# shunkenney/DPE-MVS

Hardware: AMD Instinct MI355X
Metric: depth-map Mpixels/sec (9-view 1600x1200 PatchMatch) at 1/2/4/8 GPUs; L1 vs ref (higher is better)
Workload: dtype f32; 1 GPU; DTU-like 1600x1200, 9 src views, full-res REFINE_ITER pass + geometric consistency (BASELINE configs[2]); width=1600, height=1200, num_images=10, parallelism=reference-image sharding x1

## Files before the change

### dpe-mvs_amd/csrc/dpe_mvs.hip

```cpp
#include <hip/hip_runtime.h>
#include <rocprofiler-sdk-roctx/roctx.h>
#include <algorithm>
#include <cmath>
#include <cstdio>
#include <cstring>
#include <string>
#include <atomic>
#include <map>
#include <memory>
#include <mutex>
#include <utility>
#include <vector>

#include "pass_kernels.h"
#include "pass_refine.h"
#include "pass_fusion.h"
#include "pass_sweep.h"
#include "pass_edges.h"
#include "pass_viz.h"
#include "tap_launch.h"
#include "dpe_context.h"

using namespace dpe;

static const int kDefaultXcdRows = 1;
static constexpr int kWeakLanes = 16;

namespace {
// ... 168 lines not shown
    pc.vc[v].b[2] = (float)(sK8 * trel[2]);
  }
  pc.kinv0 = (float)(1.0 / rK0);
  pc.kinv4 = (float)(1.0 / rK4);
  pc.kc2 = (float)(rK2 / rK0);
  pc.kc5 = (float)(rK5 / rK4);
  const float angle = 45.0f / pc.P.rotate_time;
  pc.gn_cos = (float)cos((double)angle * M_PI / 180.f);
  pc.gn_sin = (float)sin((double)angle * M_PI / 180.f);
  pc.gn_thr = (float)cos((double)(angle / 2.0f) * M_PI / 180.0f);
  const double sr = tan((double)(angle / 2.0f) * M_PI / 180.0f) * 20;
  const int sri = (sr != sr) ? 0 : (int)sr;
  pc.gn_shift = sri < 1 ? 1 : sri;
  pc.half_rows = std::min(pc.H, 2 * 16 * (((pc.H / 2) + 15) / 16));
  pc.weak_nn = pc.P.weak_radius >= 0 && pc.P.weak_increment > 0 ? (2 * pc.P.weak_radius) / pc.P.weak_increment + 1 : 0;
}

#if DPE_POOL_STATS
extern "C" void dpe_dbg_pool_stats_main(unsigned long long out[24], int reset) {
  (void)hipMemcpyFromSymbol(out, HIP_SYMBOL(dpe::g_pool), sizeof(dpe::g_pool));
  if (reset) { unsigned long long z[24] = {}; (void)hipMemcpyToSymbol(HIP_SYMBOL(dpe::g_pool), z, sizeof(z)); }
}
#endif
#if DPE_LINE_STATS
extern "C" void dpe_dbg_line_stats_main(unsigned long long out[16], int reset) {
  (void)hipMemcpyFromSymbol(out, HIP_SYMBOL(dpe::g_lstat), sizeof(dpe::g_lstat));
  if (reset) { unsigned long long z[16] = {}; (void)hipMemcpyToSymbol(HIP_SYMBOL(dpe::g_lstat), z, sizeof(z)); }
}
#endif
#if DPE_GN_TIMES
// ... 1220 lines not shown
```

### dpe-mvs_amd/csrc/pass_common.h

```cpp
#pragma once
#include "device_math.h"
#include "bres_walk.h"
#include "../../include/dpe_mvs.h"

namespace dpe {

struct ViewConst { float M[9]; float b[3]; };

struct PassConst {
  int W, H, N, LW, LH;
  int half_rows;
  uint32_t seed32, salt;
  float kinv0, kinv4, kc2, kc5;
  float gn_cos, gn_sin, gn_thr;
  int gn_shift;
  uint32_t gn_shift_m;
  int weak_nn;
  DpePatchMatchParams P;
  DpeCamera cams[DPE_MAX_IMAGES];
  ViewConst vc[DPE_MAX_IMAGES];
};

struct DevBufs {
  const float4* imgq[DPE_MAX_IMAGES];
  const uint8_t* img8; uint32_t img8_view;
  const uint8_t* img16; uint32_t img16_view;
  const uint8_t* imgp; uint32_t imgp_view;
  const float* depth[DPE_MAX_IMAGES];
  const float* ref;
  float4* planes; float4* planes_snap; float4* fit_plane;
  const float4* planes0;
  float* costs; float* costs_snap; float* complex_;
  uint32_t* sel; uint32_t* sel_snap;
  uint8_t* weak; uint8_t* weak_rel; uint8_t* vw;
  short2* nb; short2* nearest; short2* edge_neigh; short2* lab_bound;
  int* radius;
  const uint8_t* edge; const uint8_t* edge_low; const int* label;
  unsigned long long* cnt;
  unsigned long long* phase;
  int xcd_rows;
};

#ifndef DPE_DIAG
#define DPE_DIAG 0
#endif
#ifndef DPE_UNCLAMPED
#define DPE_UNCLAMPED 1
#endif
#define DPE_POOL_STATS (((DPE_DIAG) >> 4) & 1)
#define DPE_PHASE_PROF ((DPE_DIAG) & 1)
#define DPE_LINE_STATS (((DPE_DIAG) >> 1) & 1)
#define DPE_WEAK_STATS (((DPE_DIAG) >> 2) & 1)
#define DPE_GN_TIMES (((DPE_DIAG) >> 3) & 1)
#define DPE_FAKE_GATHER (((DPE_DIAG) >> 5) & 1)
#define DPE_GN_ONCE (((DPE_DIAG) >> 6) & 1)
#if DPE_PHASE_PROF
#define PHASE_BEGIN() uint64_t ph_t_ = __builtin_readcyclecounter(), ph_acc_[16] = {}
#define PHASE(k)                                                                    \
  do {                                                                              \
    const uint64_t n_ = __builtin_readcyclecounter();                               \
    ph_acc_[k] += n_ - ph_t_;                                                       \
    ph_t_ = n_;                                                                     \
// ... 150 lines not shown
    q1 = 2.0f * u32_to_uniform(rng_word(rs, w)) - 1.0f;
    q2 = 2.0f * u32_to_uniform(rng_word(rs, w + 1)) - 1.0f;
    s = q1 * q1 + q2 * q2;
    w += 2;
  }
  const float sq = __builtin_sqrtf(1.0f - s);
  d.n[0] = 2.0f * q1 * sq; d.n[1] = 2.0f * q2 * sq; d.n[2] = 1.0f - 2.0f * s;
  d.u_pert = u32_to_uniform(rng_word(rs, w));
  d.w_angles = w + 1;
  return d;
}
DEV void refine_angle(const Rng& rs, uint32_t w_angles, int k, float pert, float* s, float* c) {
  const float a = (u32_to_uniform(rng_word(rs, w_angles + (uint32_t)k)) - 0.5f) * pert;
  d_sincosf(a, s, c);
}
DEV float4 random_normal_from(const DpeCamera& c, int px, int py, const float* n0, float depth) {
  float4 n = make_float4(n0[0], n0[1], n0[2], 0.0f);
  const float4 vd = view_direction(c, px, py, depth);
  if (n.x * vd.x + n.y * vd.y + n.z * vd.z > 0.0f) { n.x = -n.x; n.y = -n.y; n.z = -n.z; }
  normalize3(n);
  return n;
}
DEV float4 perturbed_normal_from(const DpeCamera& c, int px, int py, const float4& normal, const float* sc) {
  const float4 vd = view_direction(c, px, py, 1.0f);
  const float s1 = sc[0], c1 = sc[1], s2 = sc[2], c2 = sc[3], s3 = sc[4], c3 = sc[5];
  const float R0 = c2 * c3, R1 = c3 * s1 * s2 - c1 * s3, R2 = s1 * s3 + c1 * c3 * s2;
  const float R3 = c2 * s3, R4 = c1 * c3 + s1 * s2 * s3, R5 = c1 * s2 * s3 - c3 * s1;
  const float R6 = -s2, R7 = c2 * s1, R8 = c1 * c2;
  float4 np = make_float4(R0 * normal.x + R1 * normal.y + R2 * normal.z,
                          R3 * normal.x + R4 * normal.y + R5 * normal.z,
                          R6 * normal.x + R7 * normal.y + R8 * normal.z, normal.w);
  if (np.x * vd.x + np.y * vd.y + np.z * vd.z >= 0.0f) np = normal;
  normalize3(np);
  return np;
}

struct Homog { float h[9]; };
DEV Homog make_homography(const PassConst& pc, int v, const float4& pl) {
  const float iw = 1.0f / pl.w;
  const float qx = pl.x * iw, qy = pl.y * iw, qz = pl.z * iw;
  const float g0 = qx * pc.kinv0;
  const float g1 = qy * pc.kinv4;
  const float g2 = __builtin_fmaf(-qx, pc.kc2, __builtin_fmaf(-qy, pc.kc5, qz));
  const ViewConst& vc = pc.vc[v];
  Homog H;
  H.h[0] = __builtin_fmaf(-vc.b[0], g0, vc.M[0]);
  H.h[1] = __builtin_fmaf(-vc.b[0], g1, vc.M[1]);
  H.h[2] = __builtin_fmaf(-vc.b[0], g2, vc.M[2]);
  H.h[3] = __builtin_fmaf(-vc.b[1], g0, vc.M[3]);
// ... 245 lines not shown

template <int U8> DEV float sample_src(const DevBufs& B, int v, int W, int H, float Qx, float Qy, float iz) {
  if constexpr (U8 != TEX_F32) return sample_quad8<U8>(tex_base<U8>(B) + (size_t)v * tex_view<U8>(B), W, H, Qx, Qy, iz);
  else return sample_quad(B.imgq[v], W, H, Qx, Qy, iz);
}

DEV float depth_texel(const float* d, int W, int H, float x, float y) {
  return ref_texel(d, W, H, f2i(x), f2i(y));
}

DEV float bilateral_weight(int i, int j, float pix, float cpix, float ss, float sc) {
  const float xd = (float)i, yd = (float)j;
  const float sd = __builtin_sqrtf(xd * xd + yd * yd);
  const float cd = __builtin_fabsf(pix - cpix);
  return d_expf(-sd / (2.0f * ss * ss) - cd / (2.0f * sc * sc));
}

DEV void ncc_pre(float s_ref, float s_rr, float s_w, float& inv, float& mref, float& var_ref) {
  inv = 1.0f / s_w;
  mref = s_ref * inv;
  const float mrr = s_rr * inv;
  var_ref = mrr - mref * mref;
}
DEV float ncc_finalize_pre(float inv, float mref, float var_ref, float s_src, float s_ss, float s_rs) {
  s_src *= inv; s_ss *= inv; s_rs *= inv;
  const float var_src = s_ss - s_src * s_src;
  if (var_ref < 1e-5f || var_src < 1e-5f) return 2.0f;
  const float cov = s_rs - mref * s_src;
  const float vrs = __builtin_sqrtf(var_ref * var_src);
  return __builtin_fmaxf(0.0f, __builtin_fminf(2.0f, 1.0f - cov / vrs));
// ... 76 lines not shown
DEV float ncc_old_generic(const PassConst& pc, const DevBufs& B, int px, int py, int v, const float4& pl) {
  const Homog H = make_homography(pc, v, pl);
  count_work(B, 1, 0);
  if (center_outside(pc, v, H, px, py)) return 2.0f;
  const float rc = ref_texel(B.ref, pc.W, pc.H, px, py);
  return patch_ncc_generic<U8>(pc, B, v, H, px, py, rc, pc.P.strong_radius, pc.P.strong_increment);
}

struct Patch36 {
  float w[36], wr[36];
  float s_ref, s_rr, s_w;
  int px, py;
};
DEV void make_patch36(Patch36& P, const PassConst& pc, const DevBufs& B, int px, int py) {
  const int W = pc.W, Hh = pc.H;
  const float ss = pc.P.sigma_spatial, sc = pc.P.sigma_color;
  const float rc = ref_texel(B.ref, W, Hh, px, py);
  P.px = px; P.py = py;
  float s_ref = 0, s_rr = 0, s_w = 0;
#pragma unroll
  for (int a = 0; a < 6; ++a) {
    const int i = -5 + 2 * a;
    float r_ref = 0, r_rr = 0, r_w = 0;
#pragma unroll
    for (int b = 0; b < 6; ++b) {
      const int j = -5 + 2 * b;
      const float rp = ref_texel(B.ref, W, Hh, px + i, py + j);
      const float w = bilateral_weight(i, j, rp, rc, ss, sc);
      const float wr = w * rp;
      r_ref = r_ref + wr;
      r_rr = __builtin_fmaf(wr, rp, r_rr);
      r_w = r_w + w;
      P.w[a * 6 + b] = w;
      P.wr[a * 6 + b] = wr;
    }
    s_ref += r_ref; s_rr += r_rr; s_w += r_w;
  }
  P.s_ref = s_ref; P.s_rr = s_rr; P.s_w = s_w;
}
template <int U8>
DEV void patch36_taps(const Patch36& P, const PassConst& pc, const DevBufs& B, int v, const Homog& H0, float* acc) {
  const int W = pc.W, Hh = pc.H;
  const Homog H = scale_cols(H0);
// ... 159 lines not shown
```

### dpe-mvs_amd/csrc/pass_refine.h

```cpp
#pragma once
#include "pass_common.h"

namespace dpe {

DEV void wave_sync() {
  __builtin_amdgcn_fence(__ATOMIC_RELEASE, "wavefront");
  __builtin_amdgcn_wave_barrier();
  __builtin_amdgcn_fence(__ATOMIC_ACQUIRE, "wavefront");
}

template <int S>
DEV void patch_lds_build(float* pw, const PassConst& pc, const DevBufs& B, int px, int py, int t) {
  constexpr int R = (36 + S - 1) / S;
  const float rc = ref_texel(B.ref, pc.W, pc.H, px, py);
  float rp[R];
#pragma unroll
  for (int r = 0; r < R; ++r) {
    const int k = t + r * S < 36 ? t + r * S : 35;
    rp[r] = ref_texel(B.ref, pc.W, pc.H, px - 5 + 2 * (k / 6), py - 5 + 2 * (k % 6));
  }
#pragma unroll
  for (int r = 0; r < R; ++r) {
    const int k = t + r * S;
    if (k >= 36) break;
    const int i = -5 + 2 * (k / 6), j = -5 + 2 * (k % 6);
    const float w = bilateral_weight(i, j, rp[r], rc, pc.P.sigma_spatial, pc.P.sigma_color);
    pw[2 * k] = w;
    pw[2 * k + 1] = w * rp[r];
    pw[72 + k] = rp[r];
  }
}
DEV void patch_lds_pre(const float* pw, float& p_inv, float& p_mref, float& p_var) {
  float a_ref = 0, a_rr = 0, a_w = 0;
#pragma unroll
  for (int a = 0; a < 6; ++a) {
    float r_ref = 0, r_rr = 0, r_w = 0;
#pragma unroll
    for (int b = 0; b < 6; ++b) {
      const float w = pw[2 * (a * 6 + b)], wr = pw[2 * (a * 6 + b) + 1], rp = pw[72 + a * 6 + b];
      r_ref = r_ref + wr;
      r_rr = __builtin_fmaf(wr, rp, r_rr);
// ... 150 lines not shown
template <int U8>
DEV float ncc_old_any(bool fast, const float* pw, float s_ref, float s_rr, float s_w, int px, int py,
                      const PassConst& pc, const DevBufs& B, int v, const float4& pl) {
  if (fast) return ncc_old_lds<U8>(pw, s_ref, s_rr, s_w, px, py, pc, B, v, pl);
  return ncc_old_generic<U8>(pc, B, px, py, v, pl);
}

DEV void baseline_and_weights(const PassConst& pc, uint32_t sel, const uint8_t* vw, float& base_line, float& weight_normal,
                              int& valid) {
  const DpeCamera& c0 = pc.cams[0];
  base_line = 0.0f; weight_normal = 0.0f; valid = 0;
  for (int si = 1; si < pc.N; ++si) {
    const int vi = si - 1;
    if (isSet(sel, vi)) {
      weight_normal += vw[vi];
      const DpeCamera& cs = pc.cams[si];
      const float d0 = c0.c[0] - cs.c[0], d1 = c0.c[1] - cs.c[1], d2 = c0.c[2] - cs.c[2];
      const float tv = d0 * d0 + d1 * d1 + d2 * d2;
      base_line += __builtin_sqrtf(tv);
      valid++;
    }
  }
}

DEV uint8_t d2w_class(const PassConst& pc, const float* pcs, uint64_t is_peak) {
  const int radius = 30;
  const int peak_count = __popcll(is_peak);
  int min_peak = 0;
  float min_cost = 2.0f;
  for (uint64_t m = is_peak; m; m &= m - 1) {
    const int i = __builtin_ctzll(m);
    if (pcs[i] < min_cost) { min_peak = i; min_cost = pcs[i]; }
  }
  uint8_t cls;
// ... 22 lines not shown
DEV long border_pixel(long i, int W, int H) {
  constexpr int m = kD2WMargin;
  if (W <= 2 * m || H <= 2 * m) return i;
  const long top = (long)m * W;
  if (i < top) return i;
  if (i < 2 * top) return (long)(H - m) * W + (i - top);
  const long r = i - 2 * top;
  const int row = m + (int)(r / (2 * m)), c = (int)(r % (2 * m));
  return (long)row * W + (c < m ? c : W - 2 * m + c);
}
template <int U8, bool LR = false>
__global__ void __launch_bounds__(64 * kBwD2W, kTapWaves) k_depth_to_weak(const PassConst* __restrict__ pcp, DevBufs B) {
  __shared__ float s_patch[kBwD2W][108];
  __shared__ float s_pc[kBwD2W][64];
  __shared__ float s_lr[kBwD2W][11];
  const PassConst& pc = *pcp;
  const int wave = threadIdx.x >> 6, lane = threadIdx.x & 63;
  const int W = pc.W, H = pc.H;
  const long pix = (long)xcd_remap(blockIdx.x, gridDim.x, B.xcd_rows * 16 * ((pc.W + kBwD2W - 1) / kBwD2W)) * kBwD2W + wave;
  if (pix >= (long)W * H) return;
  const int x = (int)(pix % W), y = (int)(pix / W);
  const int center = (int)pix;
  const int min_margin = kD2WMargin;
  if (x < min_margin || y < min_margin || x >= W - min_margin || y >= H - min_margin) {
    if (lane == 0) B.weak[center] = DPE_UNKNOWN;
    return;
  }
  const DpeCamera& c0 = pc.cams[0];
  const float4 op = transform_normal_ref(c0, B.planes[center]);
  const float od = op.w;
  if (od == 0) { if (lane == 0) B.weak[center] = DPE_UNKNOWN; return; }
  PHASE_BEGIN();
  const uint32_t sel = B.sel[center];
  const uint8_t* vw = B.vw + (size_t)DPE_MAX_IMAGES * center;
  float base_line, weight_normal; int valid;
  baseline_and_weights(pc, sel, vw, base_line, weight_normal, valid);
  if (valid == 0) { if (lane == 0) B.weak[center] = DPE_UNKNOWN; return; }
// ... 29 lines not shown
          if constexpr (LR) lr += (c * vw[vi]);
          if (pc.P.geom_consistency) {
            const float g = pc.P.geom_factor * geom_cost_at(pc, B, x, y, si, fw);
            tcst += g;
            if constexpr (LR) lr += (g * vw[vi]);
          }
          PHASE(2);
          p_cost += (tcst * vw[vi]);
        }
      }
      p_cost /= weight_normal;
      val = lane == kNow ? p_cost : MINo(2.0f, p_cost);
      lr /= weight_normal;
    }
    s_pc[wave][lane] = val;
    if (LR && lane >= radius - 5 && lane <= radius + 5) s_lr[wave][lane - (radius - 5)] = lr;
  }
  wave_sync();
  PHASE(3);
  const float* pcs = s_pc[wave];
  const bool pk = lane >= 2 && lane < 59 && pcs[lane - 1] > pcs[lane] && pcs[lane + 1] > pcs[lane];
  const uint64_t is_peak = __ballot(pk);
  PHASE(4);
  PHASE_END(3);
  if (lane != 0) return;
  B.weak[center] = d2w_class(pc, pcs, is_peak);
  if (!lr_pix) return;
  float min_cost = 2.0f, best_depth = od;
  for (int pd = -5; pd <= 5; ++pd) {
    const float p_depth = c0.K[0] * base_line / (disp + (float)pd);
    if (p_depth < pc.P.depth_min || p_depth > pc.P.depth_max) continue;
    const float tcv = s_lr[wave][pd + 5];
    if (tcv < min_cost) { min_cost = tcv; best_depth = p_depth; }
  }
  if ((double)(pcs[kNow] - min_cost) > 0.1) B.planes[center].w = best_depth;
}

constexpr int kLrPix = 4;
template <int U8>
__global__ void __launch_bounds__(64 * kBwLR, kTapWaves) k_local_refine_jobs(const PassConst* __restrict__ pcp, DevBufs B,
                                                                                     int border) {
  constexpr int BW = kBwLR;
  __shared__ float s_patch[BW][kLrPix][108];
  __shared__ float s_sum[BW][kLrPix][3];
  __shared__ float4 s_hyp[BW][kLrPix][12];
// ... 180 lines not shown
```

### dpe-mvs_amd/csrc/pass_sweep.h

```cpp
#pragma once
#include "pass_common.h"
#include "pass_refine.h"
#include "lds_layout.h"

namespace dpe {

template <int MODE> constexpr int list_count() { return MODE == 0 ? 4 : 1; }
template <int MODE> DEV int list_rows(const PassConst& pc) { return MODE == 1 ? pc.H : pc.half_rows; }
template <int MODE> DEV int list_key(const PassConst& pc, const DevBufs& B, int x, int y) {
  if constexpr (MODE == 2) return (((x + y) & 1) == 0 && B.weak_rel[y * pc.W + x] == 0) ? 0 : -1;
  const bool wk = B.weak[y * pc.W + x] == DPE_WEAK;
  if constexpr (MODE == 1) return wk ? 0 : -1;
  else return (((x + y) & 1) << 1) | (wk ? 1 : 0);
}
template <int MODE>
__global__ void k_list_count(const PassConst* __restrict__ pcp, DevBufs B, int* __restrict__ row_counts) {
  constexpr int NL = list_count<MODE>();
  const PassConst& pc = *pcp;
  const int wave = threadIdx.x >> 6, lane = threadIdx.x & 63;
  const int y = blockIdx.x * 4 + wave, rows = list_rows<MODE>(pc);
  if (y >= rows) return;
  int cnt[NL];
  for (int j = 0; j < NL; ++j) cnt[j] = 0;
  for (int x0 = 0; x0 < pc.W; x0 += 64) {
// ... 288 lines not shown
      }
      return cmp;
    }
    default: {
      if (!(x < W - 1)) return -1;
      const int right_near = center + 1; costMin = costs[right_near]; cmp = right_near;
      for (int i = 0; i < 3; ++i) {
        if (x < W - 2 - i && y > i) { const int pt = right_near + (1 + i) - (1 + i) * W; if (costs[pt] < costMin) { costMin = costs[pt]; cmp = pt; } }
        if (x < W - 2 - i && y < H - 1 - i) { const int pt = right_near + (1 + i) + (1 + i) * W; if (costs[pt] < costMin) { costMin = costs[pt]; cmp = pt; } }
      }
      return cmp;
    }
  }
}

constexpr int kTailJobs = 16;
template <int P, int C> using StrongCarveT = lds::StrongCarve<P, C, kTailJobs>;
__host__ __device__ inline int strong_lds_per_wave(int P, int C, int nv) {
  return P == 4 && C == 16 ? StrongCarveT<4, 16>::total(nv) : StrongCarveT<8, 8>::total(nv);
}

template <int P>
DEV bool job_decode(const int* cnt, int j, int& p, int& r) {
  r = j;
#pragma unroll
  for (int q = 0; q < P; ++q) {
    if (r < cnt[q]) { p = q; return true; }
    r -= cnt[q];
  }
  return false;
}

constexpr int kBwStrong = 2;
template <int U8, bool EDGE>
__global__ void __launch_bounds__(64 * kBwStrong, kTapWaves) k_strong_coop(const PassConst* __restrict__ pcp, DevBufs B, int iter,
                                                     const int* __restrict__ list, const int* __restrict__ nlist_p) {
  extern __shared__ float4 lds4[];
  float* lds = (float*)lds4;
  const int nlist = *nlist_p;
  constexpr int C = EDGE ? 16 : 8;
  constexpr int P = 64 / C;
  const PassConst& pc = *pcp;
  const int wave = threadIdx.x >> 6, lane = threadIdx.x & 63;
  const int ps = lane / C, c = lane % C;
  const int W = pc.W, nv = pc.N - 1;
  const DpeCamera& c0 = pc.cams[0];
  const int wbase = (xcd_remap(blockIdx.x, gridDim.x, B.xcd_rows * 16) * kBwStrong + wave) * P;
  if (wbase >= nlist) return;
  const int gi = wbase + ps;
  const bool active = gi < nlist;
  const int center = active ? list[gi] : 0;
  const int x = center % W, y = center / W;
  using SC = StrongCarveT<P, C>;
  float* wl = lds + (size_t)wave * SC::total(nv);
  float4* hyp_all = (float4*)(wl + SC::hyp());
  float* pw_all = wl + SC::patch();
// ... 70 lines not shown
      while (m) {
        const int t = __builtin_ctz(m);
        if (same(cpl[t], me)) { a = t; break; }
        m &= m - 1;
      }
      al[r] = a;
    }
  }
  wave_sync();
  if (active) {
    alias[c] = al[0];
    if (c == 0) alias[C] = al[1];
  }
  wave_sync();
  PHASE(1);
  if (c == 0) {
    int n = 0;
    if (active) {
      for (int k = 0; k <= C; ++k) if (alias[k] == k) slots[n++] = k;
      if (fast) patch_lds_pre(pw, sums_all[ps * 4 + 0], sums_all[ps * 4 + 1], sums_all[ps * 4 + 2]);
    }
    misc[SC::MI_JOBS] = n;
  }
  wave_sync();
  PHASE(2);
  {
    int cnt[P], S = 0;
#pragma unroll
    for (int q = 0; q < P; ++q) { cnt[q] = ib_all[q * ibs + SC::IB_MISC + 1]; S += cnt[q]; }
    int q, r;
    const int total = S * nv, tail = total & 63;
    const bool split = fast && tail > 0 && tail <= kTailJobs;
    POOL_STAT(0, total);
    const int jend = split ? total - tail : total;
    for (int j = lane; j < jend; j += 64) {
      job_decode<P>(cnt, j % S, q, r);
      const int* iq = ib_all + q * ibs;
      const int slot = iq[SC::ib_slots(nv) + r], v = j / S + 1;
      const int cq = list[wbase + q];
      const int qx = cq % W, qy = cq / W;
      const float4 pl = cpl_all[q * (C + 1) + slot];
      const float* sm = sums_all + q * 4;
      cost_all[(q * (C + 1) + slot) * nv + v - 1] =
          ncc_old_any<U8>(fast, pw_all + q * 108, sm[0], sm[1], sm[2], qx, qy, pc, B, v, pl);
    }
    if (split) {
      float* tb = wl + SC::tail(nv);
      const int rpp = 64 / tail >= 6 ? 1 : 2, npc = 6 / rpp;
      if (lane < tail * npc) {
        const int j = jend + lane / npc, a0 = (lane % npc) * rpp;
        job_decode<P>(cnt, j % S, q, r);
        const int slot = ib_all[q * ibs + SC::ib_slots(nv) + r], v = j / S + 1;
        const int cq = list[wbase + q];
        const int qx = cq % W, qy = cq / W;
        const Homog H = make_homography(pc, v, cpl_all[q * (C + 1) + slot]);
        if (!center_outside(pc, v, H, qx, qy)) {
          const bool fr = rcp_range_ok(H, (float)(qx - 5), (float)(qx + 5), (float)(qy - 5), (float)(qy + 5));
          for (int a = a0; a < a0 + rpp; ++a) {
            float* r3 = tb + ((lane / npc) * 6 + a) * 3;
            if (fr) lds_row<U8, true>(pw_all + q * 108, qx, qy, pc, B, v, H, a, r3);
            else lds_row<U8, false>(pw_all + q * 108, qx, qy, pc, B, v, H, a, r3);
          }
        }
      }
      wave_sync();
      if (lane < tail) {
        const int j = jend + lane;
        job_decode<P>(cnt, j % S, q, r);
        const int slot = ib_all[q * ibs + SC::ib_slots(nv) + r], v = j / S + 1;
        const int cq = list[wbase + q];
        const Homog H = make_homography(pc, v, cpl_all[q * (C + 1) + slot]);
        float cst = 2.0f;
        if (center_outside(pc, v, H, cq % W, cq / W)) {
          count_work(B, 1, 0);
        } else {
          count_work(B, 1, 36);
          float s_src = 0, s_ss = 0, s_rs = 0;
          for (int a = 0; a < 6; ++a) {
            const float* r3 = tb + (lane * 6 + a) * 3;
            s_src += r3[0]; s_ss += r3[1]; s_rs += r3[2];
          }
          const float* sm = sums_all + q * 4;
          cst = ncc_finalize_pre(sm[0], sm[1], sm[2], s_src, s_ss, s_rs);
        }
        cost_all[(q * (C + 1) + slot) * nv + v - 1] = cst;
      }
    }
  }
  wave_sync();
  PHASE(3);
  if (active) {
    for (int sl = c; sl <= C; sl += C) {
      const int a = alias[sl];
      if (a >= 0 && a != sl)
        for (int v = 0; v < nv; ++v) cost[sl * nv + v] = cost[a * nv + v];
    }
  }
  wave_sync();
  PHASE(4);
  if (active && c < 8) {
    if constexpr (EDGE) {
      const int d = c;
// ... 36 lines not shown
    }
    for (int v = c; v < nv; v += C) {
      float prior = 0.0f;
#pragma unroll
      for (int i = 0; i < 4; ++i) if (nfl[i]) prior += isSet(nsv[i], v) == 1 ? 0.9f : 0.1f;
      sp[v] = view_prob_raw(cst, v, cost_threshold) * prior;
    }
  }
  wave_sync();
  PHASE(6);
  Rng rs;
  rng_init(rs, (uint32_t)center, pc.seed32, STREAM_ITER_BASE + 4 * iter + 0, pc.salt);
  view_sample_coop(sp, (int*)ref, nv, c, C, active, rs, vwl, B.vw + (size_t)center * DPE_MAX_IMAGES);
  PHASE(12);
  uint32_t tsv = 0; float wnorm = 0.0f;
  if (c == 0) {
    int ns = 0;
    if (active) {
      rng_seek(rs, 15);
      for (int i = 0; i < nv; ++i) if (vwl[i] > 0) { setBit(tsv, i); wnorm += vwl[i]; sel_list[ns++] = i; }
      sums_all[ps * 4 + 3] = wnorm;
    }
    misc[SC::MI_NSEL] = ns;
  }
  wave_sync();
  PHASE(7);
  const int nsel = active ? misc[SC::MI_NSEL] : 0;
  if (active && c < 8) {
    float wn = 0.0f;
    for (int i = 0; i < nv; ++i) wn += vwl[i];
    float f = 0.0f;
    for (int j = 0; j < nv; ++j) { const int w = vwl[j]; if (w > 0) f += w * cst(c, j); }
    fc[c] = f / wn;
  }
  wave_sync();
  PHASE(8);
  float cost_now = 0.0f, cost_written = 0.0f, depth_now = 0.0f;
  float4 pnow = make_float4(0, 0, 0, 0);
// ... 11 lines not shown
    cost_now /= wnorm;
    cost_written = cost_now;
    B.costs[center] = cost_now;
    depth_now = depth_from_plane(c0, curp, x, y);
    pnow = curp;
    const int f = fin[mi];
    if (f >= 0) {
      const float4 cand = planes_s[posl[f]];
      const float db = depth_from_plane(c0, cand, x, y);
      if (db >= pc.P.depth_min && db <= pc.P.depth_max && fc[mi] < cost_now) {
        depth_now = db; pnow = cand; cost_now = fc[mi]; B.sel[center] = tsv;
      }
    }
  }
  wave_sync();
  if (active && c == 0) {
    const float dmin = pc.P.depth_min, dmax = pc.P.depth_max;
    const float depth_rand = rnd[0] * (dmax - dmin) + dmin;
    const float4 prand = random_normal_from(c0, x, y, rnd + 1, depth_now);
    const float dminp = (1 - 0.02f) * depth_now, dmaxp = (1 + 0.02f) * depth_now;
    const float depth_perturbed = rnd[4] * (dmaxp - dminp) + dminp;
    const float4 ppert = perturbed_normal_from(c0, x, y, pnow, rnd + 5);
    float4 h0 = pnow, h1 = prand, h2 = prand, h3 = ppert, h4 = pnow;
    h0.w = dist2origin(c0, x, y, depth_rand, h0);
    h1.w = dist2origin(c0, x, y, depth_now, h1);
    h2.w = dist2origin(c0, x, y, depth_rand, h2);
    h3.w = dist2origin(c0, x, y, depth_now, h3);
    h4.w = dist2origin(c0, x, y, depth_perturbed, h4);
    hyp[0] = h0; hyp[1] = h1; hyp[2] = h2; hyp[3] = h3; hyp[4] = h4;
  }
  wave_sync();
  PHASE(9);
  {
    int cnt[P];
#pragma unroll
    for (int q = 0; q < P; ++q) cnt[q] = 5 * ib_all[q * ibs + SC::IB_MISC];
    POOL_STAT(1, [&] { int t = 0; for (int q = 0; q < P; ++q) t += cnt[q]; return t; }());
    int q, r;
    for (int j = lane; job_decode<P>(cnt, j, q, r); j += 64) {
      const int* iq = ib_all + q * ibs;
      const int h = r % 5, k = r / 5;
      const int cq = list[wbase + q];
      const float* sm = sums_all + q * 4;
      ref_all[(q * 5 + h) * nv + k] = ncc_old_any<U8>(fast, pw_all + q * 108, sm[0], sm[1], sm[2], cq % W, cq / W, pc,
                                                      B, iq[SC::IB_SEL + k] + 1, hyp_all[q * 5 + h]);
    }
  }
  wave_sync();
  PHASE(10);
  if (active && c < 5) {
    const int h = c;
    float tc = 0.0f;
    for (int k = 0; k < nsel; ++k) tc += vwl[sel_list[k]] * ref[h * nv + k];
    tc /= sums_all[ps * 4 + 3];
    fc[h] = tc;
    misc[SC::MI_DEPTH + h] = __float_as_int(depth_from_plane(c0, hyp[h], x, y));
  }
  wave_sync();
  PHASE(13);
  if (active && c == 0) {
    const float dmin = pc.P.depth_min, dmax = pc.P.depth_max;
// ... 645 lines not shown
```

### dpe-mvs_amd/csrc/tap_f32.hip

```cpp
#define DPE_TAP_TU 1
#include "tap_launch.h"
#include "pass_refine.h"
#include "pass_sweep.h"

namespace dpe {

void launch_strong_f32(bool edge, unsigned grid, size_t lds, hipStream_t s, const PassConst* dpc, const DevBufs& B,
                       int it, const int* list, const int* count) {
  constexpr int T = 64 * kBwStrong;
  if (lds > 65536) {
    static bool once = false;
    if (!once) {
      once = true;
      (void)hipFuncSetAttribute((const void*)k_strong_coop<TEX_F32, true>, hipFuncAttributeMaxDynamicSharedMemorySize, 160 * 1024);
      (void)hipFuncSetAttribute((const void*)k_strong_coop<TEX_F32, false>, hipFuncAttributeMaxDynamicSharedMemorySize, 160 * 1024);
    }
  }
  if (edge) k_strong_coop<TEX_F32, true><<<grid, T, lds, s>>>(dpc, B, it, list, count);
  else k_strong_coop<TEX_F32, false><<<grid, T, lds, s>>>(dpc, B, it, list, count);
}

void launch_depth_to_weak_f32(unsigned grid, hipStream_t s, const PassConst* dpc, const DevBufs& B) {
  k_depth_to_weak<TEX_F32, true><<<grid, 64 * kBwD2W, 0, s>>>(dpc, B);
}
// ... 6 lines not shown
      once = true;
      (void)hipFuncSetAttribute((const void*)k_local_refine_jobs<TEX_F32>, hipFuncAttributeMaxDynamicSharedMemorySize, 160 * 1024);
    }
  }
  k_local_refine_jobs<TEX_F32><<<grid, 64 * kBwLR, lds, s>>>(dpc, B, border);
}

}

#if DPE_POOL_STATS
extern "C" void dpe_dbg_pool_stats_f32(unsigned long long out[24], int reset) {
  (void)hipMemcpyFromSymbol(out, HIP_SYMBOL(dpe::g_pool), sizeof(dpe::g_pool));
  if (reset) { unsigned long long z[24] = {}; (void)hipMemcpyToSymbol(HIP_SYMBOL(dpe::g_pool), z, sizeof(z)); }
}
#endif
#if DPE_LINE_STATS
extern "C" void dpe_dbg_line_stats_f32(unsigned long long out[16], int reset) {
  (void)hipMemcpyFromSymbol(out, HIP_SYMBOL(dpe::g_lstat), sizeof(dpe::g_lstat));
  if (reset) { unsigned long long z[16] = {}; (void)hipMemcpyToSymbol(HIP_SYMBOL(dpe::g_lstat), z, sizeof(z)); }
}
#endif
```

### dpe-mvs_amd/csrc/tap_launch.hip

```cpp
#define DPE_TAP_TU 1
#include "tap_launch.h"
#include "pass_refine.h"
#include "pass_sweep.h"

namespace dpe {

void launch_strong(bool edge, int cls, unsigned grid, size_t lds, hipStream_t s, const PassConst* dpc,
                   const DevBufs& B, int it, const int* list, const int* count) {
  constexpr int T = 64 * kBwStrong;
  if (lds > 65536) {
    static bool once = false;
    if (!once) {
      once = true;
      (void)hipFuncSetAttribute((const void*)k_strong_coop<kTexStrong, true>, hipFuncAttributeMaxDynamicSharedMemorySize, 160 * 1024);
      (void)hipFuncSetAttribute((const void*)k_strong_coop<kTexStrong, false>, hipFuncAttributeMaxDynamicSharedMemorySize, 160 * 1024);
    }
  }
  if (cls == IMG_F32) { launch_strong_f32(edge, grid, lds, s, dpc, B, it, list, count); return; }
  if (edge) k_strong_coop<kTexStrong, true><<<grid, T, lds, s>>>(dpc, B, it, list, count);
  else k_strong_coop<kTexStrong, false><<<grid, T, lds, s>>>(dpc, B, it, list, count);
}

void launch_depth_to_weak(int cls, long L, hipStream_t s, const PassConst* dpc, const DevBufs& B) {
  const unsigned g = (unsigned)((L + kBwD2W - 1) / kBwD2W);
// ... 14 lines not shown
      (void)hipFuncSetAttribute((const void*)k_local_refine_jobs<kTexLR>, hipFuncAttributeMaxDynamicSharedMemorySize, 160 * 1024);
    }
  }
  if (cls == IMG_F32) { launch_local_refine_f32(g, lds, border, s, dpc, B); return; }
  k_local_refine_jobs<kTexLR><<<g, 64 * kBwLR, lds, s>>>(dpc, B, border);
}

}

#if DPE_POOL_STATS
extern "C" void dpe_dbg_pool_stats_tap(unsigned long long out[24], int reset) {
  (void)hipMemcpyFromSymbol(out, HIP_SYMBOL(dpe::g_pool), sizeof(dpe::g_pool));
  if (reset) { unsigned long long z[24] = {}; (void)hipMemcpyToSymbol(HIP_SYMBOL(dpe::g_pool), z, sizeof(z)); }
}
#endif
#if DPE_LINE_STATS
extern "C" void dpe_dbg_line_stats_tap(unsigned long long out[16], int reset) {
  (void)hipMemcpyFromSymbol(out, HIP_SYMBOL(dpe::g_lstat), sizeof(dpe::g_lstat));
  if (reset) { unsigned long long z[16] = {}; (void)hipMemcpyToSymbol(HIP_SYMBOL(dpe::g_lstat), z, sizeof(z)); }
}
#endif
```

Before: 30.68 Mpix/s.

## Precompute spatial weights and baselines, spread per-pixel serial work across lanes, widen tail split

Several independent changes. The host now precomputes the bilateral spatial term table and the per-view baseline lengths into PassConst, so the exp and sqrt inputs are no longer recomputed per tap or per pixel. Depth-to-weak caches candidate depths in LDS instead of recomputing a division. The strong cooperative kernel spreads work that lane 0 of each group did serially (slot compaction, selected-view list, building 5 hypotheses) across the group's lanes using ballot and popcount. The tail-job split is generalised into a helper that handles up to 32 leftover jobs and is also applied to the hypothesis-cost pool. These add shuffles and extra LDS use and more code paths, with A/B macros left in to disable each piece.

```diff
diff --git a/dpe-mvs_amd/csrc/dpe_mvs.hip b/dpe-mvs_amd/csrc/dpe_mvs.hip
--- a/dpe-mvs_amd/csrc/dpe_mvs.hip
+++ b/dpe-mvs_amd/csrc/dpe_mvs.hip
@@ -12,6 +12,7 @@
 #include <utility>
 #include <vector>
 
+#include "pass_tables.h"
 #include "pass_kernels.h"
 #include "pass_refine.h"
 #include "pass_fusion.h"
@@ -210,6 +211,8 @@
   pc.gn_shift = sri < 1 ? 1 : sri;
   pc.half_rows = std::min(pc.H, 2 * 16 * (((pc.H / 2) + 15) / 16));
   pc.weak_nn = pc.P.weak_radius >= 0 && pc.P.weak_increment > 0 ? (2 * pc.P.weak_radius) / pc.P.weak_increment + 1 : 0;
+  for (int v = 1; v < pc.N; ++v) pc.base_len[v] = baseline_length(rc.c, pc.cams[v].c);
+  build_spat36(pc.P.sigma_spatial, pc.spat36);
 }
 
 #if DPE_POOL_STATS
diff --git a/dpe-mvs_amd/csrc/pass_common.h b/dpe-mvs_amd/csrc/pass_common.h
--- a/dpe-mvs_amd/csrc/pass_common.h
+++ b/dpe-mvs_amd/csrc/pass_common.h
@@ -16,6 +16,8 @@
   int gn_shift;
   uint32_t gn_shift_m;
   int weak_nn;
+  float base_len[DPE_MAX_IMAGES];
+  float spat36[36];
   DpePatchMatchParams P;
   DpeCamera cams[DPE_MAX_IMAGES];
   ViewConst vc[DPE_MAX_IMAGES];
@@ -46,6 +48,9 @@
 #endif
 #ifndef DPE_UNCLAMPED
 #define DPE_UNCLAMPED 1
+#endif
+#ifndef DPE_AB_OFF
+#define DPE_AB_OFF 0
 #endif
 #define DPE_POOL_STATS (((DPE_DIAG) >> 4) & 1)
 #define DPE_PHASE_PROF ((DPE_DIAG) & 1)
@@ -226,15 +231,16 @@
   const float a = (u32_to_uniform(rng_word(rs, w_angles + (uint32_t)k)) - 0.5f) * pert;
   d_sincosf(a, s, c);
 }
-DEV float4 random_normal_from(const DpeCamera& c, int px, int py, const float* n0, float depth) {
+DEV float4 random_normal_vd(const float4& vd, const float* n0) {
   float4 n = make_float4(n0[0], n0[1], n0[2], 0.0f);
-  const float4 vd = view_direction(c, px, py, depth);
   if (n.x * vd.x + n.y * vd.y + n.z * vd.z > 0.0f) { n.x = -n.x; n.y = -n.y; n.z = -n.z; }
   normalize3(n);
   return n;
 }
-DEV float4 perturbed_normal_from(const DpeCamera& c, int px, int py, const float4& normal, const float* sc) {
-  const float4 vd = view_direction(c, px, py, 1.0f);
+DEV float4 random_normal_from(const DpeCamera& c, int px, int py, const float* n0, float depth) {
+  return random_normal_vd(view_direction(c, px, py, depth), n0);
+}
+DEV float4 perturbed_normal_vd(const float4& vd, const float4& normal, const float* sc) {
   const float s1 = sc[0], c1 = sc[1], s2 = sc[2], c2 = sc[3], s3 = sc[4], c3 = sc[5];
   const float R0 = c2 * c3, R1 = c3 * s1 * s2 - c1 * s3, R2 = s1 * s3 + c1 * c3 * s2;
   const float R3 = c2 * s3, R4 = c1 * c3 + s1 * s2 * s3, R5 = c1 * s2 * s3 - c3 * s1;
@@ -245,6 +251,9 @@
   if (np.x * vd.x + np.y * vd.y + np.z * vd.z >= 0.0f) np = normal;
   normalize3(np);
   return np;
+}
+DEV float4 perturbed_normal_from(const DpeCamera& c, int px, int py, const float4& normal, const float* sc) {
+  return perturbed_normal_vd(view_direction(c, px, py, 1.0f), normal, sc);
 }
 
 struct Homog { float h[9]; };
@@ -520,6 +529,14 @@
   const float sd = __builtin_sqrtf(xd * xd + yd * yd);
   const float cd = __builtin_fabsf(pix - cpix);
   return d_expf(-sd / (2.0f * ss * ss) - cd / (2.0f * sc * sc));
+}
+
+DEV float bilateral_weight36(const PassConst& pc, int k, float pix, float cpix) {
+  const float sc = pc.P.sigma_color;
+  if constexpr ((DPE_AB_OFF) & 2)
+    return bilateral_weight(-5 + 2 * (k / 6), -5 + 2 * (k % 6), pix, cpix, pc.P.sigma_spatial, sc);
+  const float cd = __builtin_fabsf(pix - cpix);
+  return d_expf(pc.spat36[k] - cd / (2.0f * sc * sc));
 }
 
 DEV void ncc_pre(float s_ref, float s_rr, float s_w, float& inv, float& mref, float& var_ref) {
@@ -626,7 +643,6 @@
 };
 DEV void make_patch36(Patch36& P, const PassConst& pc, const DevBufs& B, int px, int py) {
   const int W = pc.W, Hh = pc.H;
-  const float ss = pc.P.sigma_spatial, sc = pc.P.sigma_color;
   const float rc = ref_texel(B.ref, W, Hh, px, py);
   P.px = px; P.py = py;
   float s_ref = 0, s_rr = 0, s_w = 0;
@@ -638,7 +654,7 @@
     for (int b = 0; b < 6; ++b) {
       const int j = -5 + 2 * b;
       const float rp = ref_texel(B.ref, W, Hh, px + i, py + j);
-      const float w = bilateral_weight(i, j, rp, rc, ss, sc);
+      const float w = bilateral_weight36(pc, a * 6 + b, rp, rc);
       const float wr = w * rp;
       r_ref = r_ref + wr;
       r_rr = __builtin_fmaf(wr, rp, r_rr);
diff --git a/dpe-mvs_amd/csrc/pass_refine.h b/dpe-mvs_amd/csrc/pass_refine.h
--- a/dpe-mvs_amd/csrc/pass_refine.h
+++ b/dpe-mvs_amd/csrc/pass_refine.h
@@ -23,8 +23,7 @@
   for (int r = 0; r < R; ++r) {
     const int k = t + r * S;
     if (k >= 36) break;
-    const int i = -5 + 2 * (k / 6), j = -5 + 2 * (k % 6);
-    const float w = bilateral_weight(i, j, rp[r], rc, pc.P.sigma_spatial, pc.P.sigma_color);
+    const float w = bilateral_weight36(pc, k, rp[r], rc);
     pw[2 * k] = w;
     pw[2 * k + 1] = w * rp[r];
     pw[72 + k] = rp[r];
@@ -205,10 +204,13 @@
     const int vi = si - 1;
     if (isSet(sel, vi)) {
       weight_normal += vw[vi];
-      const DpeCamera& cs = pc.cams[si];
-      const float d0 = c0.c[0] - cs.c[0], d1 = c0.c[1] - cs.c[1], d2 = c0.c[2] - cs.c[2];
-      const float tv = d0 * d0 + d1 * d1 + d2 * d2;
-      base_line += __builtin_sqrtf(tv);
+      if constexpr ((DPE_AB_OFF) & 1) {
+        const DpeCamera& cs = pc.cams[si];
+        const float d0 = c0.c[0] - cs.c[0], d1 = c0.c[1] - cs.c[1], d2 = c0.c[2] - cs.c[2];
+        const float tv = d0 * d0 + d1 * d1 + d2 * d2;
+        base_line += __builtin_sqrtf(tv);
+      } else
+        base_line += pc.base_len[si];
       valid++;
     }
   }
@@ -261,13 +263,14 @@
   __shared__ float s_patch[kBwD2W][108];
   __shared__ float s_pc[kBwD2W][64];
   __shared__ float s_lr[kBwD2W][11];
+  __shared__ float s_ld[kBwD2W][11];
   const PassConst& pc = *pcp;
   const int wave = threadIdx.x >> 6, lane = threadIdx.x & 63;
   const int W = pc.W, H = pc.H;
   const long pix = (long)xcd_remap(blockIdx.x, gridDim.x, B.xcd_rows * 16 * ((pc.W + kBwD2W - 1) / kBwD2W)) * kBwD2W + wave;
   if (pix >= (long)W * H) return;
-  const int x = (int)(pix % W), y = (int)(pix / W);
   const int center = (int)pix;
+  const int x = center % W, y = center / W;
   const int min_margin = kD2WMargin;
   if (x < min_margin || y < min_margin || x >= W - min_margin || y >= H - min_margin) {
     if (lane == 0) B.weak[center] = DPE_UNKNOWN;
@@ -327,7 +330,10 @@
       lr /= weight_normal;
     }
     s_pc[wave][lane] = val;
-    if (LR && lane >= radius - 5 && lane <= radius + 5) s_lr[wave][lane - (radius - 5)] = lr;
+    if (LR && lane >= radius - 5 && lane <= radius + 5) {
+      s_lr[wave][lane - (radius - 5)] = lr;
+      s_ld[wave][lane - (radius - 5)] = p_depth;
+    }
   }
   wave_sync();
   PHASE(3);
@@ -341,7 +347,7 @@
   if (!lr_pix) return;
   float min_cost = 2.0f, best_depth = od;
   for (int pd = -5; pd <= 5; ++pd) {
-    const float p_depth = c0.K[0] * base_line / (disp + (float)pd);
+    const float p_depth = ((DPE_AB_OFF) & 8) ? c0.K[0] * base_line / (disp + (float)pd) : s_ld[wave][pd + 5];
     if (p_depth < pc.P.depth_min || p_depth > pc.P.depth_max) continue;
     const float tcv = s_lr[wave][pd + 5];
     if (tcv < min_cost) { min_cost = tcv; best_depth = p_depth; }
diff --git a/dpe-mvs_amd/csrc/pass_sweep.h b/dpe-mvs_amd/csrc/pass_sweep.h
--- a/dpe-mvs_amd/csrc/pass_sweep.h
+++ b/dpe-mvs_amd/csrc/pass_sweep.h
@@ -2,6 +2,7 @@
 #include "pass_common.h"
 #include "pass_refine.h"
 #include "lds_layout.h"
+#include "pool_tail.h"
 
 namespace dpe {
 
@@ -326,7 +327,7 @@
   }
 }
 
-constexpr int kTailJobs = 16;
+constexpr int kTailJobs = kTailLdsJobs;
 template <int P, int C> using StrongCarveT = lds::StrongCarve<P, C, kTailJobs>;
 __host__ __device__ inline int strong_lds_per_wave(int P, int C, int nv) {
   return P == 4 && C == 16 ? StrongCarveT<4, 16>::total(nv) : StrongCarveT<8, 8>::total(nv);
@@ -341,6 +342,59 @@
     r -= cnt[q];
   }
   return false;
+}
+
+struct TailJob {
+  const float* pw; const float* sm; float* out;
+  int qx, qy, v;
+  float4 pl;
+};
+#if DPE_POOL_STATS
+static __device__ unsigned long long g_tail[2][4];
+#define TAIL_STAT(k, npc) do { if ((threadIdx.x & 63) == 0) atomicAdd(&g_tail[k][(npc) == 6 ? 0 : (npc) == 3 ? 1 : (npc) == 2 ? 2 : 3], 1ull); } while (0)
+#else
+#define TAIL_STAT(k, npc) do {} while (0)
+#endif
+template <int U8, class JobFn>
+DEV void pool_tail_split(int tail, int lane, float* tb, const PassConst& pc, const DevBufs& B, JobFn job) {
+  const TailLane tl = tail_lane(tail, lane);
+  const bool two = tail_lanes_per_job(tail) == 2;
+  TailJob J = {};
+  bool outside = true;
+  float acc[3] = {0.0f, 0.0f, 0.0f};
+  if (tl.job >= 0) {
+    J = job(tl.job);
+    const Homog H = make_homography(pc, J.v, J.pl);
+    outside = center_outside(pc, J.v, H, J.qx, J.qy);
+    if (!outside) {
+      const bool fr = rcp_range_ok(H, (float)(J.qx - 5), (float)(J.qx + 5), (float)(J.qy - 5), (float)(J.qy + 5));
+      for (int a = tl.row0; a < tl.row0 + tl.rows; ++a) {
+        float r3[3];
+        if (fr) lds_row<U8, true>(J.pw, J.qx, J.qy, pc, B, J.v, H, a, r3);
+        else lds_row<U8, false>(J.pw, J.qx, J.qy, pc, B, J.v, H, a, r3);
+        if (two && !tl.last) { acc[0] += r3[0]; acc[1] += r3[1]; acc[2] += r3[2]; }
+        else { float* t3 = tb + tail_lds_slot(tail, tl.job, a); t3[0] = r3[0]; t3[1] = r3[1]; t3[2] = r3[2]; }
+      }
+    }
+  }
+  const int below = lane > 0 ? lane - 1 : 0;
+  const float p0 = __shfl(acc[0], below), p1 = __shfl(acc[1], below), p2 = __shfl(acc[2], below);
+  wave_sync();
+  if (tl.job >= 0 && tl.last) {
+    float cst = 2.0f;
+    if (outside) {
+      count_work(B, 1, 0);
+    } else {
+      count_work(B, 1, 36);
+      float s_src = two ? p0 : 0.0f, s_ss = two ? p1 : 0.0f, s_rs = two ? p2 : 0.0f;
+      for (int a = two ? 3 : 0; a < 6; ++a) {
+        const float* r3 = tb + tail_lds_slot(tail, tl.job, a);
+        s_src += r3[0]; s_ss += r3[1]; s_rs += r3[2];
+      }
+      cst = ncc_finalize_pre(J.sm[0], J.sm[1], J.sm[2], s_src, s_ss, s_rs);
+    }
+    *J.out = cst;
+  }
 }
 
 constexpr int kBwStrong = 2;
@@ -352,6 +406,8 @@
   const int nlist = *nlist_p;
   constexpr int C = EDGE ? 16 : 8;
   constexpr int P = 64 / C;
+  constexpr bool kSpread = !((DPE_AB_OFF) & 4) && U8 != TEX_F32;
+  constexpr bool kWideTails = !((DPE_AB_OFF) & 16) && U8 != TEX_F32;
   const PassConst& pc = *pcp;
   const int wave = threadIdx.x >> 6, lane = threadIdx.x & 63;
   const int ps = lane / C, c = lane % C;
@@ -452,13 +508,27 @@
   }
   wave_sync();
   PHASE(1);
-  if (c == 0) {
-    int n = 0;
-    if (active) {
-      for (int k = 0; k <= C; ++k) if (alias[k] == k) slots[n++] = k;
-      if (fast) patch_lds_pre(pw, sums_all[ps * 4 + 0], sums_all[ps * 4 + 1], sums_all[ps * 4 + 2]);
-    }
-    misc[SC::MI_JOBS] = n;
+  if constexpr (!kSpread) {
+    if (c == 0) {
+      int n = 0;
+      if (active) {
+        for (int k = 0; k <= C; ++k) if (alias[k] == k) slots[n++] = k;
+        if (fast) patch_lds_pre(pw, sums_all[ps * 4 + 0], sums_all[ps * 4 + 1], sums_all[ps * 4 + 2]);
+      }
+      misc[SC::MI_JOBS] = n;
+    }
+  } else {
+    const bool own = active && alias[c] == c;
+    const uint32_t bits = (uint32_t)(__ballot(own) >> (lane - c)) & ((1u << C) - 1u);
+    if (own) slots[__popc(bits & ((1u << c) - 1u))] = c;
+    if (c == 0) {
+      int n = __popc(bits);
+      if (active) {
+        if (alias[C] == C) slots[n++] = C;
+        if (fast) patch_lds_pre(pw, sums_all[ps * 4 + 0], sums_all[ps * 4 + 1], sums_all[ps * 4 + 2]);
+      }
+      misc[SC::MI_JOBS] = n;
+    }
   }
   wave_sync();
   PHASE(2);
@@ -468,9 +538,18 @@
     for (int q = 0; q < P; ++q) { cnt[q] = ib_all[q * ibs + SC::IB_MISC + 1]; S += cnt[q]; }
     int q, r;
     const int total = S * nv, tail = total & 63;
-    const bool split = fast && tail > 0 && tail <= kTailJobs;
+    constexpr int kMaxTail = kWideTails ? kTailMaxJobs : kTailLdsJobs;
+    const bool split = fast && tail > 0 && tail <= kMaxTail;
     POOL_STAT(0, total);
+    if (tail > 0) TAIL_STAT(0, split ? tail_lanes_per_job(tail) : 1);
     const int jend = split ? total - tail : total;
+    auto cv_job = [&](int j) {
+      job_decode<P>(cnt, j % S, q, r);
+      const int slot = ib_all[q * ibs + SC::ib_slots(nv) + r], v = j / S + 1;
+      const int cq = list[wbase + q];
+      return TailJob{pw_all + q * 108, sums_all + q * 4, cost_all + (q * (C + 1) + slot) * nv + v - 1,
+                     cq % W, cq / W, v, cpl_all[q * (C + 1) + slot]};
+    };
     for (int j = lane; j < jend; j += 64) {
       job_decode<P>(cnt, j % S, q, r);
       const int* iq = ib_all + q * ibs;
@@ -482,48 +561,7 @@
       cost_all[(q * (C + 1) + slot) * nv + v - 1] =
           ncc_old_any<U8>(fast, pw_all + q * 108, sm[0], sm[1], sm[2], qx, qy, pc, B, v, pl);
     }
-    if (split) {
-      float* tb = wl + SC::tail(nv);
-      const int rpp = 64 / tail >= 6 ? 1 : 2, npc = 6 / rpp;
-      if (lane < tail * npc) {
-        const int j = jend + lane / npc, a0 = (lane % npc) * rpp;
-        job_decode<P>(cnt, j % S, q, r);
-        const int slot = ib_all[q * ibs + SC::ib_slots(nv) + r], v = j / S + 1;
-        const int cq = list[wbase + q];
-        const int qx = cq % W, qy = cq / W;
-        const Homog H = make_homography(pc, v, cpl_all[q * (C + 1) + slot]);
-        if (!center_outside(pc, v, H, qx, qy)) {
-          const bool fr = rcp_range_ok(H, (float)(qx - 5), (float)(qx + 5), (float)(qy - 5), (float)(qy + 5));
-          for (int a = a0; a < a0 + rpp; ++a) {
-            float* r3 = tb + ((lane / npc) * 6 + a) * 3;
-            if (fr) lds_row<U8, true>(pw_all + q * 108, qx, qy, pc, B, v, H, a, r3);
-            else lds_row<U8, false>(pw_all + q * 108, qx, qy, pc, B, v, H, a, r3);
-          }
-        }
-      }
-      wave_sync();
-      if (lane < tail) {
-        const int j = jend + lane;
-        job_decode<P>(cnt, j % S, q, r);
-        const int slot = ib_all[q * ibs + SC::ib_slots(nv) + r], v = j / S + 1;
-        const int cq = list[wbase + q];
-        const Homog H = make_homography(pc, v, cpl_all[q * (C + 1) + slot]);
-        float cst = 2.0f;
-        if (center_outside(pc, v, H, cq % W, cq / W)) {
-          count_work(B, 1, 0);
-        } else {
-          count_work(B, 1, 36);
-          float s_src = 0, s_ss = 0, s_rs = 0;
-          for (int a = 0; a < 6; ++a) {
-            const float* r3 = tb + (lane * 6 + a) * 3;
-            s_src += r3[0]; s_ss += r3[1]; s_rs += r3[2];
-          }
-          const float* sm = sums_all + q * 4;
-          cst = ncc_finalize_pre(sm[0], sm[1], sm[2], s_src, s_ss, s_rs);
-        }
-        cost_all[(q * (C + 1) + slot) * nv + v - 1] = cst;
-      }
-    }
+    if (split) pool_tail_split<U8>(tail, lane, wl + SC::tail(nv), pc, B, [&](int t) { return cv_job(jend + t); });
   }
   wave_sync();
   PHASE(3);
@@ -590,14 +628,33 @@
   view_sample_coop(sp, (int*)ref, nv, c, C, active, rs, vwl, B.vw + (size_t)center * DPE_MAX_IMAGES);
   PHASE(12);
   uint32_t tsv = 0; float wnorm = 0.0f;
-  if (c == 0) {
-    int ns = 0;
-    if (active) {
-      rng_seek(rs, 15);
-      for (int i = 0; i < nv; ++i) if (vwl[i] > 0) { setBit(tsv, i); wnorm += vwl[i]; sel_list[ns++] = i; }
-      sums_all[ps * 4 + 3] = wnorm;
-    }
-    misc[SC::MI_NSEL] = ns;
+  if constexpr (!kSpread) {
+    if (c == 0) {
+      int ns = 0;
+      if (active) {
+        rng_seek(rs, 15);
+        for (int i = 0; i < nv; ++i) if (vwl[i] > 0) { setBit(tsv, i); wnorm += vwl[i]; sel_list[ns++] = i; }
+        sums_all[ps * 4 + 3] = wnorm;
+      }
+      misc[SC::MI_NSEL] = ns;
+    }
+  } else {
+    for (int v0 = 0; v0 < nv; v0 += C) {
+      const bool on = active && v0 + c < nv && vwl[v0 + c] > 0;
+      tsv |= ((uint32_t)(__ballot(on) >> (lane - c)) & ((1u << C) - 1u)) << v0;
+    }
+    for (int v = c; v < nv; v += C)
+      if (isSet(tsv, v)) sel_list[__popc(tsv & ((1u << v) - 1u))] = v;
+    if (c == 0) {
+      if (active) {
+        rng_seek(rs, 15);
+        int wi = 0;
+        for (int i = 0; i < nv; ++i) wi += vwl[i];
+        wnorm = (float)wi;
+        sums_all[ps * 4 + 3] = wnorm;
+      }
+      misc[SC::MI_NSEL] = __popc(tsv);
+    }
   }
   wave_sync();
   PHASE(7);
@@ -639,7 +696,28 @@
     }
   }
   wave_sync();
-  if (active && c == 0) {
+  if constexpr (kSpread) {
+    const int l0 = lane - c;
+    const float4 pn = make_float4(__shfl(pnow.x, l0), __shfl(pnow.y, l0), __shfl(pnow.z, l0), __shfl(pnow.w, l0));
+    const float dn = __shfl(depth_now, l0);
+    if (active && c < 5) {
+      float4 h = pn;
+      if (c >= 1 && c <= 3) {
+        const float4 vd = view_direction(c0, x, y, c == 3 ? 1.0f : dn);
+        h = c == 3 ? perturbed_normal_vd(vd, pn, rnd + 5) : random_normal_vd(vd, rnd + 1);
+      }
+      float dep = dn;
+      if (c == 0 || c == 2) {
+        const float dmin = pc.P.depth_min, dmax = pc.P.depth_max;
+        dep = rnd[0] * (dmax - dmin) + dmin;
+      } else if (c == 4) {
+        const float dminp = (1 - 0.02f) * dn, dmaxp = (1 + 0.02f) * dn;
+        dep = rnd[4] * (dmaxp - dminp) + dminp;
+      }
+      h.w = dist2origin(c0, x, y, dep, h);
+      hyp[c] = h;
+    }
+  } else if (active && c == 0) {
     const float dmin = pc.P.depth_min, dmax = pc.P.depth_max;
     const float depth_rand = rnd[0] * (dmax - dmin) + dmin;
     const float4 prand = random_normal_from(c0, x, y, rnd + 1, depth_now);
@@ -662,7 +740,14 @@
     for (int q = 0; q < P; ++q) cnt[q] = 5 * ib_all[q * ibs + SC::IB_MISC];
     POOL_STAT(1, [&] { int t = 0; for (int q = 0; q < P; ++q) t += cnt[q]; return t; }());
     int q, r;
-    for (int j = lane; job_decode<P>(cnt, j, q, r); j += 64) {
+    int total = 0;
+#pragma unroll
+    for (int p = 0; p < P; ++p) total += cnt[p];
+    const int tail = total & 63;
+    const bool split = kWideTails && fast && tail > 0 && tail <= kTailMaxJobs;
+    if (tail > 0) TAIL_STAT(1, split ? tail_lanes_per_job(tail) : 1);
+    const int jend = split ? total - tail : total;
+    for (int j = lane; j < jend && job_decode<P>(cnt, j, q, r); j += 64) {
       const int* iq = ib_all + q * ibs;
       const int h = r % 5, k = r / 5;
       const int cq = list[wbase + q];
@@ -670,6 +755,14 @@
       ref_all[(q * 5 + h) * nv + k] = ncc_old_any<U8>(fast, pw_all + q * 108, sm[0], sm[1], sm[2], cq % W, cq / W, pc,
                                                       B, iq[SC::IB_SEL + k] + 1, hyp_all[q * 5 + h]);
     }
+    if (split)
+      pool_tail_split<U8>(tail, lane, wl + SC::tail(nv), pc, B, [&](int t) {
+        job_decode<P>(cnt, jend + t, q, r);
+        const int h = r % 5, k = r / 5;
+        const int cq = list[wbase + q];
+        return TailJob{pw_all + q * 108, sums_all + q * 4, ref_all + (q * 5 + h) * nv + k,
+                       cq % W, cq / W, ib_all[q * ibs + SC::IB_SEL + k] + 1, hyp_all[q * 5 + h]};
+      });
   }
   wave_sync();
   PHASE(10);
diff --git a/dpe-mvs_amd/csrc/pass_tables.h b/dpe-mvs_amd/csrc/pass_tables.h
--- /dev/null
+++ b/dpe-mvs_amd/csrc/pass_tables.h
@@ -0,0 +1,22 @@
+#pragma once
+#include <math.h>
+
+namespace dpe {
+
+constexpr int kSpatTaps = 36;
+
+inline void build_spat36(float ss, float* spat36) {
+  for (int k = 0; k < kSpatTaps; ++k) {
+    const float xd = (float)(-5 + 2 * (k / 6)), yd = (float)(-5 + 2 * (k % 6));
+    const float sd = sqrtf(xd * xd + yd * yd);
+    spat36[k] = -sd / (2.0f * ss * ss);
+  }
+}
+
+inline float baseline_length(const float* c0, const float* cs) {
+  const float d0 = c0[0] - cs[0], d1 = c0[1] - cs[1], d2 = c0[2] - cs[2];
+  const float tv = d0 * d0 + d1 * d1 + d2 * d2;
+  return sqrtf(tv);
+}
+
+}
diff --git a/dpe-mvs_amd/csrc/pool_tail.h b/dpe-mvs_amd/csrc/pool_tail.h
--- /dev/null
+++ b/dpe-mvs_amd/csrc/pool_tail.h
@@ -0,0 +1,35 @@
+#pragma once
+
+#if defined(__HIPCC__)
+#define TAIL_HD __host__ __device__
+#else
+#define TAIL_HD
+#endif
+
+namespace dpe {
+
+constexpr int kTailMaxJobs = 32;
+constexpr int kTailLdsJobs = 16;
+
+TAIL_HD constexpr int tail_lanes_per_job(int tail) {
+  return tail <= 10 ? 6 : tail <= kTailLdsJobs ? 3 : tail <= kTailMaxJobs ? 2 : 1;
+}
+
+struct TailLane {
+  int job;
+  int row0;
+  int rows;
+  bool last;
+};
+
+TAIL_HD constexpr TailLane tail_lane(int tail, int lane) {
+  const int npc = tail_lanes_per_job(tail), rpl = 6 / npc;
+  if (lane >= tail * npc) return TailLane{-1, 0, 0, false};
+  return TailLane{lane / npc, (lane % npc) * rpl, rpl, lane % npc == npc - 1};
+}
+
+TAIL_HD constexpr int tail_lds_slot(int tail, int job, int a) {
+  return tail_lanes_per_job(tail) == 2 ? (job * 3 + (a - 3)) * 3 : (job * 6 + a) * 3;
+}
+
+}
diff --git a/dpe-mvs_amd/csrc/tap_f32.hip b/dpe-mvs_amd/csrc/tap_f32.hip
--- a/dpe-mvs_amd/csrc/tap_f32.hip
+++ b/dpe-mvs_amd/csrc/tap_f32.hip
@@ -44,6 +44,12 @@
   if (reset) { unsigned long long z[24] = {}; (void)hipMemcpyToSymbol(HIP_SYMBOL(dpe::g_pool), z, sizeof(z)); }
 }
 #endif
+#if DPE_POOL_STATS
+extern "C" void dpe_dbg_tail_stats_f32(unsigned long long out[8], int reset) {
+  (void)hipMemcpyFromSymbol(out, HIP_SYMBOL(dpe::g_tail), sizeof(dpe::g_tail));
+  if (reset) { unsigned long long z[8] = {}; (void)hipMemcpyToSymbol(HIP_SYMBOL(dpe::g_tail), z, sizeof(z)); }
+}
+#endif
 #if DPE_LINE_STATS
 extern "C" void dpe_dbg_line_stats_f32(unsigned long long out[16], int reset) {
   (void)hipMemcpyFromSymbol(out, HIP_SYMBOL(dpe::g_lstat), sizeof(dpe::g_lstat));
diff --git a/dpe-mvs_amd/csrc/tap_launch.hip b/dpe-mvs_amd/csrc/tap_launch.hip
--- a/dpe-mvs_amd/csrc/tap_launch.hip
+++ b/dpe-mvs_amd/csrc/tap_launch.hip
@@ -52,6 +52,12 @@
   if (reset) { unsigned long long z[24] = {}; (void)hipMemcpyToSymbol(HIP_SYMBOL(dpe::g_pool), z, sizeof(z)); }
 }
 #endif
+#if DPE_POOL_STATS
+extern "C" void dpe_dbg_tail_stats_tap(unsigned long long out[8], int reset) {
+  (void)hipMemcpyFromSymbol(out, HIP_SYMBOL(dpe::g_tail), sizeof(dpe::g_tail));
+  if (reset) { unsigned long long z[8] = {}; (void)hipMemcpyToSymbol(HIP_SYMBOL(dpe::g_tail), z, sizeof(z)); }
+}
+#endif
 #if DPE_LINE_STATS
 extern "C" void dpe_dbg_line_stats_tap(unsigned long long out[16], int reset) {
   (void)hipMemcpyFromSymbol(out, HIP_SYMBOL(dpe::g_lstat), sizeof(dpe::g_lstat));
```

Result: faster. 31.27 Mpix/s (median of 6 runs) (+1.9%).
